# metacraft-labs/dvt-circuits

Measured on AMD Instinct MI355X. Metric: SP1 prover cycles/sec + proofs/hour, finalization_prove at 1/2/4/8 MI355X, higher is better.
Workload: dtype u32; 1 GPU; BASELINE configs[1] input: examples/finalization_test.json (tests/golden/finalization_example.json) through the reference's JSON -> CBOR -> SP1Stdin encoding, executed AND proven (the whole prove() call) by the finalization-shaped synthetic guest tests/guests.py:dkg_like(6180, 1545, 1): 32 shards of 2^21 RV32IM cycles; the reference's own guest ELF is prebuilt machine code and is not run (it would; stdin_bytes=2165, participants=3, curve_precompiles=False, fri_queries=100, pow_bits=16, log_blowup=1

## Files before the change

### dvt_circuits_amd/capi.py

```python
import ctypes as C
import json
import os
import subprocess

import numpy as np

HERE = os.path.dirname(os.path.abspath(__file__))
LIB_PATH = os.path.join(HERE, "libdvt_prover.so")
CSRC = os.path.join(HERE, "csrc")

DVT_OK, DVT_ERR_GUEST, DVT_ERR_INPUT, DVT_ERR_DEVICE, DVT_ERR_UNSUPPORTED, DVT_ERR_REJECTED = 0, 1, 2, 3, 4, 5
PATHS = {"default": 0, "rows": 1, "parts": 2}
SELECTORS = {"table": 0, "kernel": 1}
DVT_KEEP_NONE, DVT_KEEP_TREE, DVT_KEEP_FULL = 0, 1, 2
u32p = C.POINTER(C.c_uint32)
u8p = C.POINTER(C.c_uint8)


class DevMatrix(C.Structure):
    _fields_ = [("d_data", C.c_void_p), ("width", C.c_uint32), ("log_height", C.c_uint32)]


class HostTrace(C.Structure):
    _fields_ = [("chip_id", C.c_uint32), ("log_n", C.c_uint32), ("data", u32p)]
# ... 66 lines not shown
    lib.dvt_stage_bus_ledger_add.argtypes = [vp, vp, u32, vp, vp, u32, u32p, u32]
    lib.dvt_stage_bus_ledger_collect.argtypes = [vp, vp, u32, vp, vp, u32, u32p, u32]
    lib.dvt_stage_bus_ledger_add_tuple.argtypes = [vp, vp, u32, u32p, u32, C.c_int32, u32, u32]
    lib.dvt_stage_bus_ledger_close.argtypes = [vp, vp, u32p]
    lib.dvt_stage_bus_ledger_result.argtypes = [vp, vp, C.POINTER(BusTuple), sz, C.POINTER(sz), u32p]
    lib.dvt_stage_bus_ledger_free.argtypes = [vp, vp]
    lib.dvt_rv32_job_bus_tuples.argtypes = [vp, vp, vp, C.POINTER(BusTuple), sz, C.POINTER(sz), u32p]
    lib.dvt_debug_ledger_key.argtypes = [C.c_uint64, u32, u32, u32p]
    u64 = C.c_uint64
    lib.dvt_stage_hunt_cells.argtypes = [vp, C.c_char_p, u32, vp, vp, u32, u32p, u64, u32p, u32, u32, u32, u64, u32p, u8p]
    lib.dvt_stage_hunt_pairs.argtypes = [vp, C.c_char_p, u32, vp, vp, u32, u32p, u64, u32p, u32, u32p, u32, u32, u32, u32, u64,
                                         C.POINTER(Escape), sz, C.POINTER(u64), C.POINTER(u64)]
    lib.dvt_rv32_hunt_shard.argtypes = [vp, vp, vp, sz, u32, u64, u32p, u32, u32, u32p, u32, u32, u32, u32, u64, u32p, u8p,
                                        C.POINTER(Escape), sz, C.POINTER(u64), C.POINTER(u64)]
    lib.dvt_debug_ledger_key.restype = C.c_uint64
    lib.dvt_stage_hunt_join_new.argtypes = [vp, C.c_char_p, u64, u32p, u32, sz, sz, u32, C.POINTER(vp)]
    lib.dvt_stage_hunt_join_supply.argtypes = [vp, vp, u32, vp, vp, u32, u32p]
    lib.dvt_stage_hunt_join_add.argtypes = [vp, vp, u32, u32, vp, vp, u32, u32p, u32, u32, u32p, u32, u64]
    lib.dvt_stage_hunt_join_match.argtypes = [vp, vp, C.POINTER(JoinSummary)]
    lib.dvt_stage_hunt_join_result.argtypes = [vp, vp, C.POINTER(JoinCell), sz, C.POINTER(sz), C.POINTER(JoinCell), sz, C.POINTER(sz)]
    lib.dvt_stage_hunt_join_free.argtypes = [vp, vp]
    lib.dvt_rv32_hunt_join_job.argtypes = [vp, vp, vp, C.POINTER(JoinWindow), sz, u32p, u32, u64, u32p, u32, u32p, u32p, u64, sz, sz, u32,
                                           C.POINTER(JoinSummary), C.POINTER(JoinCell), sz, C.POINTER(sz), C.POINTER(JoinCell), sz, C.POINTER(sz)]
    lib.dvt_rv32_job_shard_chips.argtypes = [vp, sz]
    lib.dvt_rv32_job_shard_chips.restype = u32
    lib.dvt_rv32_job_shard_chip_shape.argtypes = [vp, sz, u32, u32p, u32p]
    lib.dvt_machine_setup.argtypes = [vp, C.c_char_p, C.POINTER(HostTrace), sz, C.POINTER(vp), C.POINTER(u8p), C.POINTER(sz)]
    lib.dvt_pk_free.argtypes = [vp, vp]
    lib.dvt_pk_free.restype = None
    lib.dvt_machine_prove.argtypes = [vp, vp, C.POINTER(HostTrace), sz, u32p, sz, C.POINTER(u8p), C.POINTER(sz)]
    lib.dvt_machine_verify.argtypes = [C.c_char_p, sz, C.c_char_p, sz, u32, u32, C.POINTER(C.c_char_p)]
    lib.dvt_prover_machine_verify.argtypes = [vp, C.c_char_p, sz, C.c_char_p, sz, u32, u32, C.POINTER(C.c_char_p)]
    lib.dvt_prover_verify.argtypes = [vp, C.c_char_p, sz, C.c_char_p, sz, u32, u32, C.POINTER(C.c_int32), C.POINTER(u8p), C.POINTER(sz), C.POINTER(C.c_char_p)]
    lib.dvt_prover_verify_times.argtypes = [vp, C.POINTER(C.c_double)]
    lib.dvt_stage_sponge_rows.argtypes = [vp, u32p, u32p, sz, u32p]
    lib.dvt_stage_verify_paths.argtypes = [vp, C.POINTER(PathChain), sz, u8p]
    lib.dvt_stage_multipath_nodes.argtypes = [u32, u32p, sz, u32p, sz, C.POINTER(sz)]
    lib.dvt_stage_verify_multipath.argtypes = [vp, u32, u32p, u32p, sz, u8p, u32p, u32p, sz, u32p, u8p]
    for fn in (lib.dvt_proof_compact, lib.dvt_proof_expand):
        fn.argtypes = [C.c_char_p, sz, C.c_char_p, sz, u32, u32, C.POINTER(u8p), C.POINTER(sz), C.POINTER(C.c_char_p)]
    lib.dvt_debug_compact_list_sweep.argtypes = [C.c_char_p, sz, C.c_char_p, sz, u32, u32, C.POINTER(u64), C.POINTER(u64), C.POINTER(C.c_char_p)]
    lib.dvt_last_stage_ms.argtypes = [vp, C.POINTER(C.c_float)]
    lib.dvt_setup.argtypes = [vp, C.c_char_p, sz, C.POINTER(vp), C.POINTER(u8p), C.POINTER(sz)]
    lib.dvt_execute.argtypes = [C.c_char_p, sz, C.POINTER(Buf), sz, C.c_uint64, C.POINTER(u8p), C.POINTER(sz), C.POINTER(Report), C.POINTER(C.c_char_p)]
    lib.dvt_execute_io.argtypes = [C.c_char_p, sz, C.POINTER(Buf), sz, C.c_uint64, C.POINTER(u8p), C.POINTER(sz), C.POINTER(u8p), C.POINTER(sz), C.POINTER(Report), C.POINTER(C.c_char_p)]
    lib.dvt_debug_exec_rate.argtypes = [C.c_char_p, sz, C.POINTER(Buf), sz, u32, C.c_int]
    lib.dvt_debug_exec_rate.restype = C.c_double
    lib.dvt_debug_p2_f64_selfcheck.argtypes = [u32, u32]
    lib.dvt_debug_p2_f64_selfcheck.restype = u64
    lib.dvt_debug_p2_f64_sbox_check.argtypes = [u32, u32, C.POINTER(C.c_double)]
    lib.dvt_debug_p2_f64_sbox_check.restype = u64
    lib.dvt_debug_ntt_group_check.argtypes = [u32, u32] + [C.POINTER(C.c_double)] * 3
    lib.dvt_debug_ntt_group_check.restype = u64
    lib.dvt_prove_core.argtypes = [vp, vp, C.POINTER(Buf), sz, C.POINTER(u8p), C.POINTER(sz), C.POINTER(Report)]
    lib.dvt_verify.argtypes = [C.c_char_p, sz, C.c_char_p, sz, u32, u32, C.POINTER(C.c_int32), C.POINTER(u8p), C.POINTER(sz), C.POINTER(C.c_char_p)]
    lib.dvt_rv32_prepare.argtypes = [vp, vp, C.POINTER(Buf), sz, C.POINTER(vp), C.POINTER(Report)]
    lib.dvt_rv32_prepare_part.argtypes = [vp, vp, C.POINTER(Buf), sz, sz, sz, C.POINTER(vp), C.POINTER(Report)]
    lib.dvt_rv32_header_words.restype = u32
    lib.dvt_rv32_job_exec_wait_seconds.argtypes = [vp]
    lib.dvt_rv32_job_exec_wait_seconds.restype = C.c_double
    lib.dvt_rv32_prove_job.argtypes = [vp, vp, vp, C.POINTER(u8p), C.POINTER(sz)]
    lib.dvt_job_free.argtypes = [vp, vp]
    lib.dvt_job_free.restype = None
    lib.dvt_rv32_debug_traces.argtypes = [C.c_char_p, sz, C.POINTER(Buf), sz, u32, u32, u32p, C.POINTER(u32p), C.POINTER(sz), C.POINTER(C.c_char_p)]
    lib.dvt_rv32_job_shards.argtypes = [vp]
    lib.dvt_rv32_job_shards.restype = sz
    lib.dvt_rv32_job_shard_member.argtypes = [vp, sz]
    lib.dvt_rv32_job_shard_member.restype = C.c_int
    lib.dvt_rv32_job_shard_device_rows.argtypes = [vp, sz]
    lib.dvt_rv32_job_shard_device_rows.restype = u32
    lib.dvt_rv32_job_shard_kept.argtypes = [vp, sz]
    lib.dvt_rv32_job_shard_kept.restype = C.c_int
    lib.dvt_rv32_job_shard_kept_bytes.argtypes = [vp, sz]
    lib.dvt_rv32_job_shard_kept_bytes.restype = C.c_uint64
    lib.dvt_debug_keep_plan.argtypes = [C.c_int, u64, u64, u64, u64, u64, u64, u64, C.c_int, C.c_int64, u64]
    lib.dvt_debug_keep_plan.restype = C.c_int
    lib.dvt_rv32_commit_shard.argtypes = [vp, vp, vp, sz, u32p]
    lib.dvt_rv32_challenges.argtypes = [C.c_char_p, sz, u32p, sz, u32p]
    lib.dvt_rv32_prove_shard.argtypes = [vp, vp, vp, sz, u32p, C.POINTER(u8p), C.POINTER(sz)]
    lib.dvt_rv32_assemble.argtypes = [vp, C.POINTER(C.c_char_p), C.POINTER(sz), sz, C.POINTER(u8p), C.POINTER(sz)]
    lib.dvt_rv32_debug_device_traces.argtypes = [vp, vp, vp, sz, C.POINTER(u32p), C.POINTER(sz)]
    lib.dvt_rv32_debug_poke_cell.argtypes = [vp, vp, sz, u32, u32, u32, u32]
    prof_out = [C.POINTER(u64), sz, C.POINTER(ProfileEdge), sz, C.POINTER(ProfileSyscall), sz, C.POINTER(ProfileOpcode), sz, C.POINTER(ProfileSummary)]
    lib.dvt_rv32_job_profile.argtypes = [vp, vp, vp, u32] + prof_out
    lib.dvt_execute_profile.argtypes = [C.c_char_p, sz, C.POINTER(Buf), sz, u64] + prof_out + [C.POINTER(Report), C.POINTER(C.c_char_p)]
    tree_out = [C.POINTER(CalltreeArc), sz, C.POINTER(CalltreeFunc), sz, C.POINTER(CalltreeSummary)]
    lib.dvt_rv32_job_calltree.argtypes = [vp, vp, vp, u32] + tree_out
    lib.dvt_rv32_job_calltree_times.argtypes = [vp, C.POINTER(C.c_double)]
    lib.dvt_execute_calltree.argtypes = [C.c_char_p, sz, C.POINTER(Buf), sz, u64] + tree_out + [C.POINTER(Report), C.POINTER(C.c_char_p)]
    mem_out = [C.POINTER(u64), sz, C.POINTER(MemoryPage), sz, C.POINTER(MemorySummary)]
    lib.dvt_rv32_job_memory.argtypes = [vp, vp, vp] + mem_out
    lib.dvt_execute_memory.argtypes = [C.c_char_p, sz, C.POINTER(Buf), sz, u64] + mem_out + [C.POINTER(Report), C.POINTER(C.c_char_p)]
    watch_io = [C.POINTER(WatchQuery), sz, sz, C.POINTER(WatchHit), C.POINTER(u64), C.POINTER(WatchSummary)]
    lib.dvt_rv32_job_watch.argtypes = [vp, vp, vp] + watch_io
    lib.dvt_rv32_job_watch_times.argtypes = [vp, C.POINTER(C.c_double)]
    lib.dvt_execute_watch.argtypes = [C.c_char_p, sz, C.POINTER(Buf), sz, u64, u32] + watch_io + [C.POINTER(Report), C.POINTER(C.c_char_p)]
    snap_io = [u32, u32, C.POINTER(SnapRange), sz, C.POINTER(SnapCell), C.POINTER(SnapCell), sz, C.POINTER(SnapFrame), sz, C.POINTER(SnapSummary)]
    lib.dvt_rv32_job_snapshot.argtypes = [vp, vp, vp] + snap_io
    lib.dvt_rv32_job_snapshot_times.argtypes = [vp, C.POINTER(C.c_double)]
    lib.dvt_execute_snapshot.argtypes = [C.c_char_p, sz, C.POINTER(Buf), sz, u64, u32] + snap_io + [C.POINTER(Report), C.POINTER(C.c_char_p)]
    origin_io = [u32, u32, u32, u32, u32, u32, C.POINTER(OriginNode), sz, C.POINTER(OriginEdge), sz, C.POINTER(OriginSummary)]
    lib.dvt_rv32_job_origin.argtypes = [vp, vp, vp] + origin_io
    lib.dvt_rv32_job_origin_times.argtypes = [vp, C.POINTER(C.c_double)]
    lib.dvt_execute_origin.argtypes = [C.c_char_p, sz, C.POINTER(Buf), sz, u64, u32] + origin_io + [C.POINTER(Report), C.POINTER(C.c_char_p)]
    diverge_io = [DivergePos, DivergePos, u64, u32, u32, sz, C.POINTER(DivergePair), C.POINTER(DivergePair), C.POINTER(DivergeReg), C.POINTER(DivergeSummary)]
    lib.dvt_rv32_job_diverge.argtypes = [vp, vp, vp, vp] + diverge_io
# ... 527 lines not shown
    first, last, regs, s = (DivergePair * max(keep, 1))(), (DivergePair * max(keep, 1))(), (DivergeReg * 32)(), DivergeSummary()
    rc = call(DivergePos(*start_a), DivergePos(*start_b), max_pairs, DVT_DIVERGE_REJOIN if rejoin else 0, window, keep, first, last, regs, C.byref(s))
    if rc != DVT_OK:
        return rc, None
    summary = {}
    for name, kind in DivergeSummary._fields_:
        if name in ("pad", "pad2"):
            continue
        v = getattr(s, name)
        if kind is DivergeRec:
            summary[name] = {k: int(getattr(v, k)) for k in _DIV_REC_KEYS if k != "valid"} if v.valid else None
        else:
            summary[name] = float(v) if name == "ms" else int(v)
    n = summary["n_kept"]
    return rc, dict(summary=summary, regs=[{k: int(getattr(regs[r], k)) for k in _DIV_REG_KEYS} for r in range(32)],
                    first=[{k: int(getattr(first[i], k)) for k in _DIV_PAIR_KEYS} for i in range(n)],
                    last=[{k: int(getattr(last[i], k)) for k in _DIV_PAIR_KEYS} for i in range(n)])


def execute_diverge(elf: bytes, stdin_a: bytes, stdin_b: bytes, start_a=DIVERGE_ENTRY, start_b=DIVERGE_ENTRY, max_pairs=0, rejoin=False, window=0, keep=16,
                    max_cycles=0, log_shard=21):
    lib = load()
    reps, err = (Report(), Report()), C.c_char_p()
    a, b = bytes(stdin_a), bytes(stdin_b)
    rc, got = _diverge(lambda *io: lib.dvt_execute_diverge(elf, len(elf), a, len(a), b, len(b), max_cycles, log_shard, *io, C.byref(reps[0]), C.byref(reps[1]),
                                                           C.byref(err)), start_a, start_b, max_pairs, rejoin, window, keep)
    return rc, tuple(dict(cycles=r.cycles, exit_code=r.exit_code, halted=bool(r.halted), unprovable=bool(r.unprovable)) for r in reps), got, _take_str(lib, err)


def exec_rate(elf: bytes, stdin=(), log_shard=21, trace=False) -> float:
    return float(load().dvt_debug_exec_rate(elf, len(elf), _bufs(stdin), len(stdin), log_shard, int(trace)))


def keep_plan(mode, free, total, reserve, full, tree, later, remaining=0, count_known=True, full_cap=-1, full_kept=0) -> int:
    return int(load().dvt_debug_keep_plan(mode, free, total, reserve, full, tree, later, remaining, int(bool(count_known)), full_cap, full_kept))


def p2_f64_selfcheck(n: int, seed: int) -> int:
    return int(load().dvt_debug_p2_f64_selfcheck(n, seed))


def p2_f64_sbox_check(n: int, seed: int):
    mx = (C.c_double * 4)()
    bad = load().dvt_debug_p2_f64_sbox_check(n, seed, mx)
    return int(bad), [float(v) for v in mx]


def ntt_group_check(n: int, seed: int):
    mx = [(C.c_double * 8)() for _ in range(3)]
    bad = load().dvt_debug_ntt_group_check(n, seed, *mx)
    return int(bad), {k: [float(v) for v in m] for k, m in zip(("dif", "dif_unit", "dit"), mx)}


def execute_io(elf: bytes, stdin=(), max_cycles=0):
    lib = load()
    pv, n, so, m, rep, err = u8p(), C.c_size_t(), u8p(), C.c_size_t(), Report(), C.c_char_p()
    rc = lib.dvt_execute_io(elf, len(elf), _bufs(stdin), len(stdin), max_cycles, C.byref(pv), C.byref(n), C.byref(so), C.byref(m), C.byref(rep), C.byref(err))
    out = C.string_at(pv, n.value) if pv else b""
    sout = C.string_at(so, m.value) if so else b""
    for ptr in (pv, so):
        if ptr:
            lib.dvt_free(C.cast(ptr, C.c_void_p))
    return rc, dict(cycles=rep.cycles, exit_code=rep.exit_code, halted=bool(rep.halted), unprovable=bool(rep.unprovable)), out, sout, _take_str(lib, err)


def stdin_from_json(circuit_type: str, json_bytes: bytes, auth_commitment=False) -> bytes:
    lib = load()
    out, n, err = u8p(), C.c_size_t(), C.c_char_p()
    rc = lib.dvt_stdin_from_json(circuit_type.encode(), json_bytes, len(json_bytes), int(bool(auth_commitment)), C.byref(out), C.byref(n), C.byref(err))
    if rc:
        raise DvtError(rc, _take_str(lib, err))
    b = C.string_at(out, n.value)
    lib.dvt_free(C.cast(out, C.c_void_p))
    return b


def verify(vk: bytes, proof: bytes, fri_queries=100, pow_bits=16):
    lib = load()
    ec, pv, n, why = C.c_int32(), u8p(), C.c_size_t(), C.c_char_p()
    rc = lib.dvt_verify(vk, len(vk), proof, len(proof), fri_queries, pow_bits, C.byref(ec), C.byref(pv), C.byref(n), C.byref(why))
    out = C.string_at(pv, n.value) if pv else b""
    if pv:
        lib.dvt_free(C.cast(pv, C.c_void_p))
    return rc == DVT_OK, ec.value, out, _take_str(lib, why)


def _transcode(fn, vk, proof, fri_queries, pow_bits):
    lib = load()
    out, n, why = u8p(), C.c_size_t(), C.c_char_p()
    rc = fn(vk, len(vk), proof, len(proof), fri_queries, pow_bits, C.byref(out), C.byref(n), C.byref(why))
    reason = _take_str(lib, why)
    if rc:
        raise DvtError(rc, reason)
    b = C.string_at(out, n.value)
    lib.dvt_free(C.cast(out, C.c_void_p))
    return b


def proof_compact(vk: bytes, proof: bytes, fri_queries=100, pow_bits=16) -> bytes:
    return _transcode(load().dvt_proof_compact, vk, proof, fri_queries, pow_bits)


def proof_expand(vk: bytes, proof: bytes, fri_queries=100, pow_bits=16) -> bytes:
    return _transcode(load().dvt_proof_expand, vk, proof, fri_queries, pow_bits)


# ... 627 lines not shown
```

### dvt_circuits_amd/csrc/capi_rv32.hip

```cpp
#include <algorithm>
#include <atomic>
#include <cstdio>
#include <deque>
#include <map>

#include "capi_job.h"
#include "ntt_group.cuh"
#include "poseidon2_f64.cuh"
#include "sha256.h"

using namespace dvt;
static_assert(DVT_KEEP_NONE == KEEP_NONE && DVT_KEEP_TREE == KEEP_TREE && DVT_KEEP_FULL == KEEP_FULL, "the tiers of include/dvt_prover.h");

namespace {
std::vector<std::vector<uint8_t>> collect_stdin(const dvt_buf *bufs, size_t n) {
    std::vector<std::vector<uint8_t>> v(n);
    for (size_t i = 0; i < n; i++)
        if (bufs[i].len) v[i].assign(bufs[i].data, bufs[i].data + bufs[i].len);
    return v;
}
uint8_t *dup_bytes(const std::vector<uint8_t> &v, size_t *len) {
    uint8_t *b = (uint8_t *)malloc(v.size() + 1);
    if (b && !v.empty()) memcpy(b, v.data(), v.size());
    if (len) *len = v.size();
    return b;
}
PermChallenges global_challenges(const VerifyingKey &vk, const uint32_t *headers, size_t n) {
    Challenger g;
    g.observe(vk.prep_root);
    g.observe_u32((uint32_t)n);
    for (size_t i = 0; i < n; i++) {
        const uint32_t *h = headers + i * HEADER_WORDS;
        for (uint32_t k = 0; k < 8; k++) g.observe(Fp::from_canonical(h[k]));
        g.observe_u32(N_PUB);
        for (uint32_t k = 0; k < N_PUB; k++) g.observe(Fp::from_canonical(h[8 + k] % P));
    }
    PermChallenges c;
    c.alpha = g.sample_ext();
    c.beta = g.sample_ext();
    return c;
}
void pv_digest_words(const std::vector<uint8_t> &pv, uint32_t out[8]) {
    uint8_t dg[32];
    sha256(pv.data(), pv.size(), dg);
    for (int k = 0; k < 8; k++) out[k] = dg[4 * k] | (dg[4 * k + 1] << 8) | (dg[4 * k + 2] << 16) | ((uint32_t)dg[4 * k + 3] << 24);
}
}

int dvt::same_members(dvt_prover *p, const dvt_pk *pk, const dvt_job *j) {
    const size_t G = n_members(p);
    if ((pk && pk->dev.size() != G) || (j && j->parts.size() != G)) return fail(p, DVT_ERR_INPUT, "proving key or job of a handle with other devices");
    return DVT_OK;
}

static void job_release(dvt_prover *p, dvt_job *j) {
    if (!j) return;
    for (size_t m = std::min(j->parts.size(), n_members(p)); m-- > 0;) {
        (void)turn_to(p, m);
        Member &mem = member(p, m);
// ... 1486 lines not shown
            if (kind == 2) {
                const int64_t a = ref[j], b = ref[j + dist] * wj % (int64_t)P;
                ref[j] = (a + b) % (int64_t)P; ref[j + dist] = ntg_mod(a - b);
            } else {
                const int64_t a = ref[j], b = ref[j + dist];
                ref[j] = (a + b) % (int64_t)P; ref[j + dist] = ntg_mod(a - b) * wj % (int64_t)P;
            }
        }
    }
    uint64_t bad = 0;
    for (int j = 0; j < 8; j++)
        for (int c = 0; c < 2; c++) {
            const double x = v[j][c];
            const bool sane = fabs(x) < 9e15 && x == floor(x);
            bad += !sane || ntg_mod((int64_t)x) != (c ? ntg_mod(-ref[j]) : ref[j]);
        }
    return bad;
}
}

uint64_t dvt_debug_ntt_group_check(uint32_t n, uint32_t seed, double *max_dif, double *max_dif_unit, double *max_dit) {
    uint64_t bad = 0, s = 0x9e3779b97f4a7c15ull ^ seed;
    double mx[3][8] = {};
    const int64_t lim[3] = {(int64_t)ntg::DIF_IN, (int64_t)ntg::DIF_IN, (int64_t)ntg::DIT_IN}, half = ((int64_t)P - 1) / 2;
    auto next = [&]() { s ^= s << 13; s ^= s >> 7; s ^= s << 17; return s; };
    auto uniform = [&](int64_t m) { return (int64_t)(next() % (2 * (uint64_t)m + 1)) - m; };
    int64_t in[8], tw[7];
    for (uint32_t g = 0; g < n; g++)
        for (int kind = 0; kind < 3; kind++) {
            for (int j = 0; j < 8; j++) in[j] = uniform(lim[kind]);
            for (int k = 0; k < 7; k++) tw[k] = uniform(half);
            bad += ntg_check_one(kind, in, tw, mx[kind]);
        }
    const int64_t mags[5] = {0, 1, half, (int64_t)P - 1, (int64_t)(0.52 * p2f::PD)};
    const int64_t tws[4] = {1, -1, half, -half};
    for (int kind = 0; kind < 3; kind++)
        for (int m = 0; m < 5; m++)
            for (int signs = 0; signs < 256; signs++) {
                if (m == 0 && signs) break;
                const int64_t mag = mags[m] > lim[kind] ? lim[kind] : mags[m];
                for (int j = 0; j < 8; j++) in[j] = (signs >> j) & 1 ? -mag : mag;
                for (int c = 0; c < 64 + 8; c++) {
                    for (int k = 0; k < 7; k++) {
                        const int stage = kind == 2 ? (k < 1 ? 0 : k < 3 ? 1 : 2) : (k < 4 ? 0 : k < 6 ? 1 : 2);
                        tw[k] = c < 64 ? tws[(c >> (2 * stage)) & 3] : uniform(half);
                    }
                    bad += ntg_check_one(kind, in, tw, mx[kind]);
                }
            }
    for (int k = 0; k < 8; k++) { max_dif[k] = mx[0][k]; max_dif_unit[k] = mx[1][k]; max_dit[k] = mx[2][k]; }
    return bad;
}

}
```

### dvt_circuits_amd/csrc/f64dot.cuh

```cuda
#pragma once
#include "poseidon2_f64.cuh"

namespace dvt {

struct DotAcc {
    double lo, hi;
    DVT_HD void add(double w, double vlo, double vhi) { lo = fma(w, vlo, lo); hi = fma(w, vhi, hi); }
    DVT_HD void reduce() { lo = p2f::red(lo); hi = p2f::red(hi); }
    DVT_HD Fp value() const { return Fp::raw(p2f::fix(p2f::red(fma(p2f::red(hi), 65536.0, lo)))); }
};
struct DotAcc4 {
    DotAcc c[4];
    DVT_HD DotAcc4() { for (int k = 0; k < 4; k++) c[k] = DotAcc{0.0, 0.0}; }
    DVT_HD void add(const double *w4, Fp v) {
        const double vlo = (double)(v.v & 0xffffu), vhi = (double)(v.v >> 16);
#pragma unroll
        for (int k = 0; k < 4; k++) c[k].add(w4[k], vlo, vhi);
    }
    DVT_HD void reduce() {
#pragma unroll
        for (int k = 0; k < 4; k++) c[k].reduce();
    }
    DVT_HD Fp4 value() const {
        Fp4 r;
#pragma unroll
        for (int k = 0; k < 4; k++) r.c[k] = c[k].value();
        return r;
    }
    DVT_HD void value_canonical(double out[4]) const {
#pragma unroll
        for (int k = 0; k < 4; k++) out[k] = p2f::mm(p2f::red(fma(p2f::red(c[k].hi), 65536.0, c[k].lo)), p2f::MONT_RINV);
    }
};
struct Fd4 {
    double c[4];
};
DVT_HD Fd4 operator*(const Fd4 &a, const Fd4 &b) {
    const double q0 = b.c[0] * p2f::PINV, q1 = b.c[1] * p2f::PINV, q2 = b.c[2] * p2f::PINV, q3 = b.c[3] * p2f::PINV;
    auto m = [&](int i, int j, double qj) { return p2f::mm_pre(a.c[i], b.c[j], qj); };
    Fd4 r;
    r.c[0] = fma(11.0, m(1, 3, q3) + m(2, 2, q2) + m(3, 1, q1), m(0, 0, q0));
    r.c[1] = fma(11.0, m(2, 3, q3) + m(3, 2, q2), m(0, 1, q1) + m(1, 0, q0));
    r.c[2] = fma(11.0, m(3, 3, q3), m(0, 2, q2) + m(1, 1, q1) + m(2, 0, q0));
    r.c[3] = (m(0, 3, q3) + m(1, 2, q2)) + (m(2, 1, q1) + m(3, 0, q0));
    return r;
}
DVT_HD Fd4 operator*(const Fd4 &a, double b) {
    const double bq = b * p2f::PINV;
    Fd4 r;
    for (int k = 0; k < 4; k++) r.c[k] = p2f::mm_pre(a.c[k], b, bq);
    return r;
}
DVT_HD Fd4 operator+(const Fd4 &a, const Fd4 &b) { Fd4 r; for (int k = 0; k < 4; k++) r.c[k] = a.c[k] + b.c[k]; return r; }
DVT_HD Fd4 operator-(const Fd4 &a, const Fd4 &b) { Fd4 r; for (int k = 0; k < 4; k++) r.c[k] = a.c[k] - b.c[k]; return r; }

DVT_HD double centred_from_mont(uint32_t m) { return p2f::from_mont(m); }

}
```

### dvt_circuits_amd/csrc/machine.h

```cpp
#pragma once
#include "check.cuh"
#include "stark.cuh"

namespace dvt {

struct VerifierAccess {
    const Fp4 *main_l, *main_n, *prep_l, *prep_n, *perm_l, *perm_n;
    const Fp *pubv;
    Fp4 main(int c, int r) const { return r ? main_n[c] : main_l[c]; }
    Fp4 prep(int c, int r) const { return r ? prep_n[c] : prep_l[c]; }
    Fp4 pub(int k) const { return Fp4::from_base(pubv[k]); }
    Fp4 perm(int e, int r) const {
        const Fp4 *p = (r ? perm_n : perm_l) + 4 * e;
        Fp4 acc = p[0];
        for (int k = 1; k < 4; k++) {
            Fp4 basis = Fp4::zero();
            basis.c[k] = Fp::one();
            acc += basis * p[k];
        }
        return acc;
    }
};

struct VerifierPoint {
    const Fp4 *alpha_pows, *beta_pows;
    Fp4 perm_alpha, cum_over_n, sel_first, sel_last, sel_trans;
};

struct LedgerArgs;
struct HuntArgs;
struct JoinArgs;

struct ChipDesc {
    const char *name;
    int main_w, prep_w, n_pub, n_constraints, n_interactions, max_arity;
    int perm_ext_w;
    int n_folded;
    bool perm_parts, quot_parts;
    hipError_t (*launch_perm)(hipStream_t, const PermArgs &);
    hipError_t (*launch_quotient)(hipStream_t, const QuotientArgs &);
    Fp4 (*verify_eval)(const VerifierAccess &, const VerifierPoint &);
    hipError_t (*launch_check)(hipStream_t, const CheckArgs &) = nullptr;
    hipError_t (*launch_bus)(hipStream_t, const BusArgs &) = nullptr;
    hipError_t (*launch_ledger)(hipStream_t, const LedgerArgs &) = nullptr;
    hipError_t (*launch_hunt)(hipStream_t, const HuntArgs &, unsigned row_blocks, unsigned n_candidates) = nullptr;
    hipError_t (*launch_join)(hipStream_t, const JoinArgs &, unsigned row_blocks, unsigned n_candidates) = nullptr;
    hipError_t (*launch_supply)(hipStream_t, const JoinArgs &) = nullptr;
};

struct MachineDesc {
    const char *name;
    int n_chips;
    const ChipDesc *chips;
};

constexpr int RV32_FIRST_WIDE_CHIP = 9;
const MachineDesc *machine_toy();
const MachineDesc *machine_rv32();
const MachineDesc *machine_by_name(const char *name);

#if defined(__HIPCC__)
template <class Air>
constexpr bool perm_parts_parallel() { return Air::N_INTERACTIONS > 0 && Air::N_LPARTS > 1 && Air::N_LPARTS <= PARTS_MAX; }
template <class Air>
constexpr bool quot_parts_parallel() {
    constexpr int NP = Air::N_PARTS + (Air::N_INTERACTIONS > 0 ? Air::N_LPARTS : 0);
    return NP > 2 && NP <= PARTS_MAX && Air::MAIN_W >= 128;
}
template <class Air>
hipError_t launch_perm_t(hipStream_t st, const PermArgs &a) {
    if (Air::N_INTERACTIONS == 0) return hipSuccess;
    size_t n = (size_t)1 << a.log_n;
    if constexpr (perm_parts_parallel<Air>()) {
        if (a.partial) {
            perm_rows_parts_kernel<Air><<<dim3((unsigned)((n + 255) / 256), Air::N_LPARTS), 256, 0, st>>>(a);
            sum_parts_kernel<0><<<(unsigned)((4 * n + 255) / 256), 256, 0, st>>>(a.partial, Air::N_LPARTS, 4 * n, a.totals);
            return hipGetLastError();
        }
    }
    perm_rows_kernel<Air><<<(unsigned)((n + 255) / 256), 256, 0, st>>>(a);
    return hipGetLastError();
}
template <class Air, int PART>
void launch_quotient_parts(hipStream_t st, const QuotientArgs &a, unsigned blocks) {
    constexpr int LAST = Air::N_PARTS + (Air::N_INTERACTIONS > 0 ? Air::N_LPARTS : 0) - 1;
    quotient_kernel<Air, PART><<<blocks, 256, 0, st>>>(a);
    if constexpr (PART < LAST) launch_quotient_parts<Air, PART + 1>(st, a, blocks);
}
template <class Air>
hipError_t launch_quotient_t(hipStream_t st, const QuotientArgs &a) {
    size_t m = (size_t)2 << a.log_n;
    constexpr int NP = Air::N_PARTS + (Air::N_INTERACTIONS > 0 ? Air::N_LPARTS : 0);
    if constexpr (quot_parts_parallel<Air>()) {
        if (a.partial) {
            quotient_parts_kernel<Air><<<dim3((unsigned)((m + 255) / 256), NP), 256, 0, st>>>(a);
            sum_parts_kernel<0><<<(unsigned)((4 * m + 255) / 256), 256, 0, st>>>(a.partial, NP, 4 * m, a.out);
            return hipGetLastError();
        }
    }
    launch_quotient_parts<Air, 0>(st, a, (unsigned)((m + 255) / 256));
    return hipGetLastError();
}
template <class Air>
Fp4 verify_eval_t(const VerifierAccess &ax, const VerifierPoint &pt) {
    ConstraintFolder<Air, Fp4, VerifierAccess> f(ax);
    f.alpha_pows = pt.alpha_pows;
    f.beta_pows = pt.beta_pows;
    f.perm_alpha = pt.perm_alpha;
    f.cum_over_n = pt.cum_over_n;
    f.sel_first = pt.sel_first;
    f.sel_last = pt.sel_last;
    f.sel_trans = pt.sel_trans;
    return f.run();
}
template <class Air>
constexpr ChipDesc make_chip_desc() {
    return ChipDesc{Air::NAME, Air::MAIN_W, Air::PREP_W, Air::N_PUB, Air::N_CONSTRAINTS, Air::N_INTERACTIONS,
                    Air::MAX_ARITY, PermShape<Air>::EXT_W, PermShape<Air>::N_FOLDED,
                    perm_parts_parallel<Air>(), quot_parts_parallel<Air>(), &launch_perm_t<Air>, &launch_quotient_t<Air>, &verify_eval_t<Air>};
}
template <class Air>
ChipDesc with_check_fns(ChipDesc d) {
    d.launch_check = &launch_check_t<Air>;
    d.launch_bus = &launch_bus_t<Air>;
    return d;
}
#endif

}
```

### dvt_circuits_amd/csrc/machine_rv32_wide.hip

```cpp
#include "machine.h"
#if !defined(__HIP_DEVICE_COMPILE__)
#pragma clang optimize off
#endif
#include "gen/air_rv32.inc"
#if !defined(__HIP_DEVICE_COMPILE__)
#pragma clang optimize on
#endif

#include "gen/rv32_cols.h"
static_assert(dvt::RV32_FIRST_WIDE_CHIP == RV32_CHIP_FP_OP, "machine.h RV32_FIRST_WIDE_CHIP must be the fp_op chip");

namespace dvt {
namespace {
template <int I, class A>
bool pick(int chip, ChipDesc *out) {
    if constexpr (I >= RV32_FIRST_WIDE_CHIP) {
        if (chip == I) { *out = make_chip_desc<A>(); return true; }
    }
    return false;
}
}
ChipDesc rv32_wide_chip_desc(int chip) {
    ChipDesc d{};
#define DVT_X(i, A) if (pick<i, A>(chip, &d)) return d;
    DVT_AIR_RV32_CHIPS(DVT_X)
#undef DVT_X
    return d;
}
}
```

### dvt_circuits_amd/csrc/stark.cuh

```cuda
#pragma once
#include "bb.cuh"
#include "f64dot.cuh"
#include "kernels.h"

namespace dvt {

constexpr int WHEN_ALL = 0, WHEN_FIRST = 1, WHEN_LAST = 2, WHEN_TRANS = 3;

DVT_HD Fp4 to_ext(Fp a) { return Fp4::from_base(a); }
DVT_HD Fp4 to_ext(const Fp4 &a) { return a; }

template <class Air>
struct PermShape {
    static constexpr int NB = (Air::N_INTERACTIONS + 1) / 2;
    static constexpr int EXT_W = Air::N_INTERACTIONS ? NB : 0;
    static constexpr int PHI = NB - 1;
    static constexpr int BASE_W = 4 * EXT_W;
    static constexpr int N_FOLDED = Air::N_CONSTRAINTS + (Air::N_INTERACTIONS ? NB : 0);
};

template <class Air, class TT, class Access>
struct ConstraintFolder {
    using T = TT;
    using Shape = PermShape<Air>;
// ... 126 lines not shown
        if ((j & 1) == 0) {
            pend_m = m;
            pend_d = d;
            if (j == Air::N_INTERACTIONS - 1) {
                Fp4 p = batch_value(j >> 1);
                fold(Air::N_CONSTRAINTS + (j >> 1), p * d - to_ext(m));
            }
        } else {
            Fp4 p = batch_value(j >> 1);
            Fp4 lhs = p * pend_d * d;
            Fp4 rhs = d * pend_m + pend_d * m;
            fold(Air::N_CONSTRAINTS + (j >> 1), lhs - rhs);
        }
    }

    template <int PART = -1>
    DVT_HD Fp4 run() {
        if constexpr (BASE)
            for (int k = 0; k < 4; k++) perm_alpha_c.c[k] = centred_from_mont(perm_alpha.c[k].v);
        if constexpr (PART < 0) {
            Air::constraints(*this);
            Air::interactions(*this);
        } else if constexpr (PART < Air::N_PARTS) {
            Air::template constraints_part<PART>(*this);
        } else {
            Air::template interactions_part<PART - Air::N_PARTS>(*this);
        }
        if constexpr (BASE) {
            acc += acc_d.value();
            Fp4 lc;
            for (int k = 0; k < 4; k++) lc.c[k] = Fp::raw(p2f::to_mont(acc_c.c[k]));
            acc += lc;
        }
        return acc;
    }
};

#if defined(__HIPCC__)
struct PermArgs {
    const uint32_t *main;
    const uint32_t *prep;
    const uint32_t *pub;
    uint32_t *perm;
    uint32_t *totals;
    const Fp4 *beta_pows;
    const double *beta_d;
    Fp4 perm_alpha;
    uint32_t log_n;
    uint32_t *partial = nullptr;
};
constexpr int PARTS_MAX = 32;
constexpr uint32_t PARTS_PARALLEL_LOG = 15;

template <class Air>
struct PermRowCtx {
    using T = Fp;
    const PermArgs &a;
    size_t n, row;
    Fp4 batch, total;
    __device__ PermRowCtx(const PermArgs &args, size_t r) : a(args), n((size_t)1 << args.log_n), row(r), batch(Fp4::zero()), total(Fp4::zero()) {}
    __device__ static T K(uint32_t m) { return Fp::raw(m); }
    __device__ static T KI(uint32_t canonical) { return Fp::from_canonical(canonical); }
    __device__ T main(int c, int r) const { return Fp::raw(a.main[(size_t)c * n + ((row + r) & (n - 1))]); }
    __device__ T prep(int c, int r) const { return Fp::raw(a.prep[(size_t)c * n + ((row + r) & (n - 1))]); }
    __device__ T pub(int k) const { return Fp::raw(a.pub[k]); }
    __device__ void store_ext(int extcol, const Fp4 &v) {
#pragma unroll
        for (int k = 0; k < 4; k++) a.perm[((size_t)(4 * extcol + k)) * n + row] = v.c[k].v;
    }
    __device__ void interaction(int j, int bus, int sign, int , const T &mult, const T *vals, int nv) {
        Fp4 term = Fp4::zero();
        if (!mult.is_zero()) {
            DotAcc4 s;
            for (int k = 0; k < nv; k++) {
                s.add(a.beta_d + 4 * k, vals[k]);
                if ((k & 31) == 31) s.reduce();
            }
            Fp4 d = a.perm_alpha + Fp::from_canonical((uint32_t)bus) + s.value();
            term = inv(d) * (sign > 0 ? mult : -mult);
        }
        if ((j & 1) == 0) batch = term; else batch += term;
        if ((j & 1) || j == Air::N_INTERACTIONS - 1) {
            if ((j >> 1) < PermShape<Air>::PHI) store_ext(j >> 1, batch);
            total += batch;
        }
    }
};

template <class Air>
__global__ void __launch_bounds__(256) perm_rows_kernel(PermArgs a) {
    size_t row = (size_t)blockIdx.x * blockDim.x + threadIdx.x;
    if (row >= ((size_t)1 << a.log_n)) return;
    PermRowCtx<Air> ctx(a, row);
    Air::interactions(ctx);
#pragma unroll
    for (int k = 0; k < 4; k++) a.totals[(size_t)k * ctx.n + row] = ctx.total.c[k].v;
}

template <class Air, int LP, class Ctx>
__device__ __forceinline__ void interactions_of_part(Ctx &ctx, int part) {
    if (part == LP) Air::template interactions_part<LP>(ctx);
    else if constexpr (LP + 1 < Air::N_LPARTS) interactions_of_part<Air, LP + 1>(ctx, part);
}
template <class Air>
__global__ void __launch_bounds__(256) perm_rows_parts_kernel(PermArgs a) {
    size_t row = (size_t)blockIdx.x * blockDim.x + threadIdx.x;
    if (row >= ((size_t)1 << a.log_n)) return;
    PermRowCtx<Air> ctx(a, row);
    interactions_of_part<Air, 0>(ctx, (int)blockIdx.y);
#pragma unroll
    for (int k = 0; k < 4; k++) a.partial[((size_t)blockIdx.y * 4 + k) * ctx.n + row] = ctx.total.c[k].v;
}
template <int UNUSED>
__global__ void __launch_bounds__(256) sum_parts_kernel(const uint32_t *partial, uint32_t nparts, size_t words, uint32_t *out) {
    size_t w = (size_t)blockIdx.x * blockDim.x + threadIdx.x;
    if (w >= words) return;
    Fp acc = Fp::raw(partial[w]);
    for (uint32_t p = 1; p < nparts; p++) acc = acc + Fp::raw(partial[(size_t)p * words + w]);
    out[w] = acc.v;
}

struct QuotientArgs {
    const uint32_t *main_lde;
    const uint32_t *prep_lde;
    const uint32_t *perm_lde;
    const uint32_t *pub;
    uint32_t *out;
    const Fp4 *alpha_pows;
    const Fp4 *beta_pows;
    const double *alpha_d, *beta_d;
    Fp4 perm_alpha, cum_over_n;
    Fp zinv_even, zinv_odd;
    Fp z_even, z_odd;
    Fp w_inv;
    uint32_t log_n;
    NttTables tabs;
    const uint32_t *sel = nullptr;
    uint32_t *partial = nullptr;
};

__device__ __forceinline__ void selectors_of_row(const QuotientArgs &a, size_t i, Fp *sel_first, Fp *sel_last, Fp *sel_trans) {
    const uint32_t log_m = a.log_n + 1;
    Fp x = Fp::raw(a.tabs.sh_lo[1]) * (Fp::raw(a.tabs.tw_hi[((uint32_t)i << (24 - log_m)) >> 12]) *
                                        Fp::raw(a.tabs.tw_lo[((uint32_t)i << (24 - log_m)) & 4095]));
    const Fp zh = (i & 1) ? a.z_odd : a.z_even;
    Fp d1 = x - Fp::one(), d2 = x - a.w_inv;
    Fp pinv = inv(d1 * d2);
    *sel_first = zh * (pinv * d2);
    *sel_last = zh * (pinv * d1);
    *sel_trans = d2;
}
template <int UNUSED>
__global__ void __launch_bounds__(256) selector_table_kernel(QuotientArgs a, uint32_t *out) {
    const size_t m = (size_t)2 << a.log_n;
    size_t i = (size_t)blockIdx.x * blockDim.x + threadIdx.x;
    if (i >= m) return;
    Fp f, l, t;
    selectors_of_row(a, i, &f, &l, &t);
    out[i] = f.v; out[m + i] = l.v; out[2 * m + i] = t.v;
}

// ... 81 lines not shown
```

### include/dvt_prover.h

```cpp
#ifndef DVT_PROVER_H
#define DVT_PROVER_H
#include <stddef.h>
#include <stdint.h>
#ifdef __cplusplus
extern "C" {
#endif

#define DVT_OK 0
#define DVT_ERR_GUEST 1
#define DVT_ERR_INPUT 2
#define DVT_ERR_DEVICE 3
#define DVT_ERR_UNSUPPORTED 4
#define DVT_ERR_REJECTED 5

typedef struct dvt_prover dvt_prover;
typedef struct dvt_pk dvt_pk;

int dvt_prover_create(const char *cfg_json, dvt_prover **out);
uint32_t dvt_prover_device_count(const dvt_prover *p);
int dvt_prover_device(const dvt_prover *p, uint32_t member);
void dvt_prover_destroy(dvt_prover *p);
const char *dvt_last_error(const dvt_prover *p);
void dvt_free(void *ptr);
uint32_t dvt_abi_version(void);
// ... 352 lines not shown
enum { DVT_DIV_RD = 1, DVT_DIV_RS1 = 2, DVT_DIV_RS2 = 4, DVT_DIV_MEM = 8 };
enum { DVT_DIVERGE_REJOIN = 1 };
enum { DVT_DIV_SPLIT = 1, DVT_DIV_BAD = 2, DVT_DIV_END_BOTH = 3, DVT_DIV_END_A = 4, DVT_DIV_END_B = 5, DVT_DIV_LIMIT = 6 };
typedef struct { uint32_t shard, row; } dvt_diverge_pos;
typedef struct { uint32_t valid, pc, idx, a, b, c, m_prev, pad; } dvt_diverge_rec;
typedef struct {
    uint64_t k;
    uint32_t shard_a, row_a, shard_b, row_b, idx, pc, mask, dir;
    uint32_t a_a, b_a, c_a, m_a, a_b, b_b, c_b, m_b;
    uint32_t addr_a, before_a, after_a, addr_b, before_b, after_b;
} dvt_diverge_pair;
typedef struct { uint64_t n_diff, first_diff, last_diff, last_write; uint32_t live, pad; } dvt_diverge_reg;
typedef struct {
    uint64_t n_pairs, n_data, first_data, last_data, n_load_diffs, n_store_diffs, launched_pairs, cycles_a, cycles_b;
    uint32_t reason, mask, stop_shard_a, stop_row_a, stop_shard_b, stop_row_b;
    uint32_t rejoin_shard_a, rejoin_row_a, rejoin_shard_b, rejoin_row_b, rejoin_skip_a, rejoin_skip_b;
    uint32_t n_kept, span, window, batch_pairs;
    dvt_diverge_rec stop_a, stop_b, prev_a, prev_b;
    float ms;
    uint32_t pad2;
} dvt_diverge_summary;
int dvt_rv32_job_diverge(dvt_prover *p, const dvt_pk *pk, dvt_job *job_a, dvt_job *job_b, dvt_diverge_pos start_a, dvt_diverge_pos start_b,
                         uint64_t max_pairs, uint32_t flags, uint32_t window, size_t cap_each, dvt_diverge_pair *first, dvt_diverge_pair *last,
                         dvt_diverge_reg regs[32], dvt_diverge_summary *summary);
int dvt_rv32_job_diverge_times(dvt_prover *p, double out[4]);
int dvt_execute_diverge(const uint8_t *elf, size_t elf_len, const uint8_t *stdin_a, size_t n_a, const uint8_t *stdin_b, size_t n_b, uint64_t max_cycles,
                        uint32_t log_shard_size, dvt_diverge_pos start_a, dvt_diverge_pos start_b, uint64_t max_pairs, uint32_t flags, uint32_t window,
                        size_t cap_each, dvt_diverge_pair *first, dvt_diverge_pair *last, dvt_diverge_reg regs[32], dvt_diverge_summary *summary,
                        dvt_report *report_a, dvt_report *report_b, char **err_text);
int dvt_rv32_debug_device_traces(dvt_prover *p, const dvt_pk *pk, dvt_job *job, size_t shard, uint32_t **blob,
                                 size_t *blob_words);
int dvt_rv32_debug_poke_cell(dvt_prover *p, dvt_job *job, size_t shard, uint32_t chip, uint32_t col, uint32_t row,
                             uint32_t add);
int dvt_verify(const uint8_t *vk, size_t vk_len, const uint8_t *proof, size_t proof_len, uint32_t fri_queries,
               uint32_t pow_bits, int32_t *exit_code, uint8_t **public_values, size_t *pv_len, char **reason);
int dvt_prover_verify(dvt_prover *p, const uint8_t *vk, size_t vk_len, const uint8_t *proof, size_t proof_len,
                      uint32_t fri_queries, uint32_t pow_bits, int32_t *exit_code, uint8_t **public_values,
                      size_t *pv_len, char **reason);
int dvt_proof_compact(const uint8_t *vk, size_t vk_len, const uint8_t *proof, size_t proof_len, uint32_t fri_queries,
                      uint32_t pow_bits, uint8_t **out, size_t *out_len, char **reason);
int dvt_proof_expand(const uint8_t *vk, size_t vk_len, const uint8_t *proof, size_t proof_len, uint32_t fri_queries,
                     uint32_t pow_bits, uint8_t **out, size_t *out_len, char **reason);
int dvt_debug_compact_list_sweep(const uint8_t *vk, size_t vk_len, const uint8_t *proof, size_t proof_len, uint32_t fri_queries,
                                 uint32_t pow_bits, uint64_t *n_words, uint64_t *n_accepted, char **reason);
int dvt_prover_verify_times(dvt_prover *p, double out[9]);
int dvt_debug_keep_plan(int mode, uint64_t free_bytes, uint64_t total_bytes, uint64_t reserve_bytes, uint64_t full_bytes,
                        uint64_t tree_bytes, uint64_t later_bytes, uint64_t remaining, int count_known, int64_t full_cap,
                        uint64_t full_kept);
double dvt_debug_exec_rate(const uint8_t *elf, size_t elf_len, const dvt_buf *stdin_bufs, size_t nbuf, uint32_t log_shard,
                           int trace);
uint64_t dvt_debug_p2_f64_selfcheck(uint32_t n, uint32_t seed);
uint64_t dvt_debug_p2_f64_sbox_check(uint32_t n, uint32_t seed, double *max_abs);
uint64_t dvt_debug_ntt_group_check(uint32_t n, uint32_t seed, double *max_dif, double *max_dif_unit, double *max_dit);
uint64_t dvt_debug_ledger_key(uint64_t seed, uint32_t bus, uint32_t arity, const uint32_t *values);

int dvt_stdin_from_json(const char *type, const char *json, size_t json_len, int auth_commitment, uint8_t **out,
                        size_t *out_len, char **err_text);
int dvt_json_schema_validate(const char *schema, size_t schema_len, const char *json, size_t json_len, char **err_text);

int dvt_rv32_debug_traces(const uint8_t *elf, size_t elf_len, const dvt_buf *stdin_bufs, size_t nbuf, uint32_t log_shard,
                          uint32_t shard, uint32_t *n_shards, uint32_t **blob, size_t *blob_words, char **err_text);

#ifdef __cplusplus
}
#endif
#endif
```

Measured before the change: 80.78 million guest cycles/s.

## Compute permutation interactions in f64 with paired-fraction batching for narrow chips

Adds an f64 path for the permutation (logup) row kernel on non-wide chips. Quartic-extension products and inverses are done in double-precision Montgomery arithmetic, and interactions are paired so that one extension inverse serves two fractions (d1*m2 + d2*m1)/(d1*d2). The aim is to cut the cost of per-interaction Fp4 inversions and integer Montgomery multiplies on the GPU. Wide chips keep the old integer path. It adds numerical-range risk in f64 and ships a host self-check for that.

```diff
diff --git a/dvt_circuits_amd/capi.py b/dvt_circuits_amd/capi.py
--- a/dvt_circuits_amd/capi.py
+++ b/dvt_circuits_amd/capi.py
@@ -142,6 +142,8 @@
     lib.dvt_debug_p2_f64_sbox_check.restype = u64
     lib.dvt_debug_ntt_group_check.argtypes = [u32, u32] + [C.POINTER(C.c_double)] * 3
     lib.dvt_debug_ntt_group_check.restype = u64
+    lib.dvt_debug_k45_f64_check.argtypes = [u32, u32, C.POINTER(C.c_double)]
+    lib.dvt_debug_k45_f64_check.restype = u64
     lib.dvt_prove_core.argtypes = [vp, vp, C.POINTER(Buf), sz, C.POINTER(u8p), C.POINTER(sz), C.POINTER(Report)]
     lib.dvt_verify.argtypes = [C.c_char_p, sz, C.c_char_p, sz, u32, u32, C.POINTER(C.c_int32), C.POINTER(u8p), C.POINTER(sz), C.POINTER(C.c_char_p)]
     lib.dvt_rv32_prepare.argtypes = [vp, vp, C.POINTER(Buf), sz, C.POINTER(vp), C.POINTER(Report)]
@@ -775,6 +777,12 @@
     return int(bad), {k: [float(v) for v in m] for k, m in zip(("dif", "dif_unit", "dit"), mx)}
 
 
+def k45_f64_check(n: int, seed: int):
+    mx = (C.c_double * 3)()
+    bad = load().dvt_debug_k45_f64_check(n, seed, mx)
+    return int(bad), [float(v) for v in mx]
+
+
 def execute_io(elf: bytes, stdin=(), max_cycles=0):
     lib = load()
     pv, n, so, m, rep, err = u8p(), C.c_size_t(), u8p(), C.c_size_t(), Report(), C.c_char_p()
diff --git a/dvt_circuits_amd/csrc/capi_rv32.hip b/dvt_circuits_amd/csrc/capi_rv32.hip
--- a/dvt_circuits_amd/csrc/capi_rv32.hip
+++ b/dvt_circuits_amd/csrc/capi_rv32.hip
@@ -5,6 +5,7 @@
 #include <map>
 
 #include "capi_job.h"
+#include "f64dot.cuh"
 #include "ntt_group.cuh"
 #include "poseidon2_f64.cuh"
 #include "sha256.h"
@@ -1597,4 +1598,70 @@
     return bad;
 }
 
-}
+uint64_t dvt_debug_k45_f64_check(uint32_t n, uint32_t seed, double *max_abs) {
+    uint64_t bad = 0, s = 0x9e3779b97f4a7c15ull ^ seed;
+    double mx[3] = {0, 0, 0};
+    const int64_t half = ((int64_t)P - 1) / 2;
+    auto next = [&]() { s ^= s << 13; s ^= s >> 7; s ^= s << 17; return s; };
+    auto uniform = [&](int64_t m) { return (int64_t)(next() % (2 * (uint64_t)m + 1)) - m; };
+    auto ref_of = [&](const Fd4 &a) {
+        Fp4 r;
+        for (int k = 0; k < 4; k++) r.c[k] = Fp::from_canonical((uint32_t)ntg_mod((int64_t)a.c[k]));
+        return r;
+    };
+    auto differs = [&](const Fd4 &got, const Fp4 &want, int slot) {
+        uint64_t d = 0;
+        for (int k = 0; k < 4; k++) {
+            const double x = got.c[k];
+            const bool sane = fabs(x) < 9e15 && x == floor(x);
+            d += !sane || (uint32_t)ntg_mod((int64_t)x) != want.c[k].canonical() || (fabs(x) < 1.4e14 && p2f::to_mont(x) != want.c[k].v);
+            if (sane) mx[slot] = fmax(mx[slot], fabs(x));
+        }
+        return d;
+    };
+    auto check_prod = [&](const Fd4 &a, const Fd4 &b) {
+        double am = 0, bm = 0;
+        for (int k = 0; k < 4; k++) { am = fmax(am, fabs(a.c[k])); bm = fmax(bm, fabs(b.c[k])); }
+        if (am * bm > FD4_PROD_IN) return;
+        mx[0] = fmax(mx[0], am * bm);
+        bad += differs(a * b, ref_of(a) * ref_of(b), 1);
+    };
+    auto check_inv = [&](const Fd4 &a) { bad += differs(inv(a), inv(ref_of(a)), 2); };
+    const int64_t wide = (int64_t)(6.12 * p2f::PD), mid = (int64_t)(1.02 * p2f::PD);
+    for (uint32_t t = 0; t < n; t++) {
+        Fd4 a, b;
+        for (int k = 0; k < 4; k++) { a.c[k] = (double)uniform(wide); b.c[k] = (double)uniform(mid); }
+        check_prod(a, b);
+        check_prod(b, a);
+        check_inv(b);
+        check_inv(a * b);
+        Fd4 c = b;
+        for (int k = 0; k < 4; k++) c.c[k] += (double)(uniform(16) * (int64_t)P);
+        check_inv(c);
+        check_inv(Fd4{{b.c[0], 0.0, 0.0, 0.0}});
+    }
+    const int64_t mags[7] = {0, 1, half, half + 1, (int64_t)P - 1, mid, wide};
+    for (int ma = 0; ma < 7; ma++)
+        for (int mb = 0; mb < 7; mb++)
+            for (int signs = 0; signs < 256; signs++) {
+                Fd4 a, b;
+                for (int k = 0; k < 4; k++) {
+                    a.c[k] = (double)((signs >> k) & 1 ? -mags[ma] : mags[ma]);
+                    b.c[k] = (double)((signs >> (4 + k)) & 1 ? -mags[mb] : mags[mb]);
+                }
+                check_prod(a, b);
+                if (mb == 0 && signs < 16) check_inv(a);
+            }
+    const int64_t singles[6] = {1, -1, half, -half, half + 1, -(half + 1)};
+    for (int k = 0; k < 4; k++)
+        for (int v = 0; v < 6; v++) {
+            Fd4 a = {{0.0, 0.0, 0.0, 0.0}};
+            a.c[k] = (double)singles[v];
+            check_inv(a);
+        }
+    for (int64_t z = -1; z <= 1; z++) check_inv(Fd4{{(double)(z * (int64_t)P), 0.0, (double)(-z * (int64_t)P), 0.0}});
+    for (int k = 0; k < 3; k++) max_abs[k] = mx[k];
+    return bad;
+}
+
+}
diff --git a/dvt_circuits_amd/csrc/f64dot.cuh b/dvt_circuits_amd/csrc/f64dot.cuh
--- a/dvt_circuits_amd/csrc/f64dot.cuh
+++ b/dvt_circuits_amd/csrc/f64dot.cuh
@@ -35,14 +35,16 @@
 struct Fd4 {
     double c[4];
 };
+constexpr int FD4_K = 12;
+constexpr double FD4_PROD_IN = 3.66e19;
 DVT_HD Fd4 operator*(const Fd4 &a, const Fd4 &b) {
     const double q0 = b.c[0] * p2f::PINV, q1 = b.c[1] * p2f::PINV, q2 = b.c[2] * p2f::PINV, q3 = b.c[3] * p2f::PINV;
-    auto m = [&](int i, int j, double qj) { return p2f::mm_pre(a.c[i], b.c[j], qj); };
+    auto m = [&](int i, int j, double qj) { return p2f::mm_c<FD4_K>(a.c[i], b.c[j], qj); };
     Fd4 r;
-    r.c[0] = fma(11.0, m(1, 3, q3) + m(2, 2, q2) + m(3, 1, q1), m(0, 0, q0));
-    r.c[1] = fma(11.0, m(2, 3, q3) + m(3, 2, q2), m(0, 1, q1) + m(1, 0, q0));
-    r.c[2] = fma(11.0, m(3, 3, q3), m(0, 2, q2) + m(1, 1, q1) + m(2, 0, q0));
-    r.c[3] = (m(0, 3, q3) + m(1, 2, q2)) + (m(2, 1, q1) + m(3, 0, q0));
+    r.c[0] = p2f::red(fma(11.0, m(1, 3, q3) + m(2, 2, q2) + m(3, 1, q1), m(0, 0, q0)));
+    r.c[1] = p2f::red(fma(11.0, m(2, 3, q3) + m(3, 2, q2), m(0, 1, q1) + m(1, 0, q0)));
+    r.c[2] = p2f::red(fma(11.0, m(3, 3, q3), m(0, 2, q2) + m(1, 1, q1) + m(2, 0, q0)));
+    r.c[3] = p2f::red((m(0, 3, q3) + m(1, 2, q2)) + (m(2, 1, q1) + m(3, 0, q0)));
     return r;
 }
 DVT_HD Fd4 operator*(const Fd4 &a, double b) {
@@ -54,6 +56,37 @@
 DVT_HD Fd4 operator+(const Fd4 &a, const Fd4 &b) { Fd4 r; for (int k = 0; k < 4; k++) r.c[k] = a.c[k] + b.c[k]; return r; }
 DVT_HD Fd4 operator-(const Fd4 &a, const Fd4 &b) { Fd4 r; for (int k = 0; k < 4; k++) r.c[k] = a.c[k] - b.c[k]; return r; }
 
+DVT_HD double inv_base(double a) {
+    const double ap = a * p2f::PINV;
+    const double a2 = p2f::mm_pre(a, a, ap), a3 = p2f::mm_pre(a2, a, ap);
+    const double a7 = p2f::mm_pre(p2f::mm(a3, a3), a, ap);
+    const double a7p = a7 * p2f::PINV;
+    double r = p2f::mm_pre(a7, a7, a7p);
+#pragma unroll
+    for (int i = 0; i < 9; i++) {
+        r = p2f::mm(r, r); r = p2f::mm(r, r); r = p2f::mm(r, r);
+        r = p2f::mm_pre(r, a7, a7p);
+    }
+    return r;
+}
+DVT_HD Fd4 inv(const Fd4 &a) {
+    using namespace p2f;
+    const double A0 = red(a.c[0]), B0 = red(a.c[1]), A1 = red(a.c[2]), B1 = red(a.c[3]);
+    const double A2_0 = fma(11.0, mm(A1, A1), mm(A0, A0)), A2_1 = 2.0 * mm(A0, A1);
+    const double B2_0 = fma(11.0, mm(B1, B1), mm(B0, B0)), B2_1 = 2.0 * mm(B0, B1);
+    const double D0 = fma(-11.0, B2_1, A2_0), D1 = A2_1 - B2_0;
+    const double ni = inv_base(fma(-11.0, mm(D1, D1), mm(D0, D0)));
+    const double nip = ni * PINV;
+    const double I0 = mm_pre(D0, ni, nip), I1 = -mm_pre(D1, ni, nip);
+    const double I0p = I0 * PINV, I1p = I1 * PINV;
+    Fd4 r;
+    r.c[0] = fma(11.0, mm_pre(A1, I1, I1p), mm_pre(A0, I0, I0p));
+    r.c[2] = mm_pre(A0, I1, I1p) + mm_pre(A1, I0, I0p);
+    r.c[1] = -fma(11.0, mm_pre(B1, I1, I1p), mm_pre(B0, I0, I0p));
+    r.c[3] = -(mm_pre(B0, I1, I1p) + mm_pre(B1, I0, I0p));
+    return r;
+}
+
 DVT_HD double centred_from_mont(uint32_t m) { return p2f::from_mont(m); }
 
 }
diff --git a/dvt_circuits_amd/csrc/machine.h b/dvt_circuits_amd/csrc/machine.h
--- a/dvt_circuits_amd/csrc/machine.h
+++ b/dvt_circuits_amd/csrc/machine.h
@@ -67,18 +67,21 @@
     constexpr int NP = Air::N_PARTS + (Air::N_INTERACTIONS > 0 ? Air::N_LPARTS : 0);
     return NP > 2 && NP <= PARTS_MAX && Air::MAIN_W >= 128;
 }
-template <class Air>
+struct ChipKind { static constexpr bool K4_F64 = true; };
+struct WideChipKind { static constexpr bool K4_F64 = false; };
+template <class Air, class Kind>
 hipError_t launch_perm_t(hipStream_t st, const PermArgs &a) {
+    constexpr bool F64 = Kind::K4_F64;
     if (Air::N_INTERACTIONS == 0) return hipSuccess;
     size_t n = (size_t)1 << a.log_n;
     if constexpr (perm_parts_parallel<Air>()) {
         if (a.partial) {
-            perm_rows_parts_kernel<Air><<<dim3((unsigned)((n + 255) / 256), Air::N_LPARTS), 256, 0, st>>>(a);
+            perm_rows_parts_kernel<Air, F64><<<dim3((unsigned)((n + 255) / 256), Air::N_LPARTS), 256, 0, st>>>(a);
             sum_parts_kernel<0><<<(unsigned)((4 * n + 255) / 256), 256, 0, st>>>(a.partial, Air::N_LPARTS, 4 * n, a.totals);
             return hipGetLastError();
         }
     }
-    perm_rows_kernel<Air><<<(unsigned)((n + 255) / 256), 256, 0, st>>>(a);
+    perm_rows_kernel<Air, F64><<<(unsigned)((n + 255) / 256), 256, 0, st>>>(a);
     return hipGetLastError();
 }
 template <class Air, int PART>
@@ -113,11 +116,11 @@
     f.sel_trans = pt.sel_trans;
     return f.run();
 }
-template <class Air>
+template <class Air, class Kind = ChipKind>
 constexpr ChipDesc make_chip_desc() {
     return ChipDesc{Air::NAME, Air::MAIN_W, Air::PREP_W, Air::N_PUB, Air::N_CONSTRAINTS, Air::N_INTERACTIONS,
                     Air::MAX_ARITY, PermShape<Air>::EXT_W, PermShape<Air>::N_FOLDED,
-                    perm_parts_parallel<Air>(), quot_parts_parallel<Air>(), &launch_perm_t<Air>, &launch_quotient_t<Air>, &verify_eval_t<Air>};
+                    perm_parts_parallel<Air>(), quot_parts_parallel<Air>(), &launch_perm_t<Air, Kind>, &launch_quotient_t<Air>, &verify_eval_t<Air>};
 }
 template <class Air>
 ChipDesc with_check_fns(ChipDesc d) {
diff --git a/dvt_circuits_amd/csrc/machine_rv32_wide.hip b/dvt_circuits_amd/csrc/machine_rv32_wide.hip
--- a/dvt_circuits_amd/csrc/machine_rv32_wide.hip
+++ b/dvt_circuits_amd/csrc/machine_rv32_wide.hip
@@ -15,7 +15,7 @@
 template <int I, class A>
 bool pick(int chip, ChipDesc *out) {
     if constexpr (I >= RV32_FIRST_WIDE_CHIP) {
-        if (chip == I) { *out = make_chip_desc<A>(); return true; }
+        if (chip == I) { *out = make_chip_desc<A, WideChipKind>(); return true; }
     }
     return false;
 }
diff --git a/dvt_circuits_amd/csrc/stark.cuh b/dvt_circuits_amd/csrc/stark.cuh
--- a/dvt_circuits_amd/csrc/stark.cuh
+++ b/dvt_circuits_amd/csrc/stark.cuh
@@ -202,13 +202,18 @@
 constexpr int PARTS_MAX = 32;
 constexpr uint32_t PARTS_PARALLEL_LOG = 15;
 
-template <class Air>
+template <class Air, bool F64 = true>
 struct PermRowCtx {
     using T = Fp;
     const PermArgs &a;
     size_t n, row;
     Fp4 batch, total;
-    __device__ PermRowCtx(const PermArgs &args, size_t r) : a(args), n((size_t)1 << args.log_n), row(r), batch(Fp4::zero()), total(Fp4::zero()) {}
+    Fd4 perm_alpha_c, pend_d;
+    double pend_m = 0.0;
+    __device__ PermRowCtx(const PermArgs &args, size_t r) : a(args), n((size_t)1 << args.log_n), row(r), batch(Fp4::zero()), total(Fp4::zero()) {
+        if constexpr (F64)
+            for (int k = 0; k < 4; k++) perm_alpha_c.c[k] = centred_from_mont(a.perm_alpha.c[k].v);
+    }
     __device__ static T K(uint32_t m) { return Fp::raw(m); }
     __device__ static T KI(uint32_t canonical) { return Fp::from_canonical(canonical); }
     __device__ T main(int c, int r) const { return Fp::raw(a.main[(size_t)c * n + ((row + r) & (n - 1))]); }
@@ -218,7 +223,56 @@
 #pragma unroll
         for (int k = 0; k < 4; k++) a.perm[((size_t)(4 * extcol + k)) * n + row] = v.c[k].v;
     }
+    __device__ static Fp4 to_mont4(const Fd4 &v) {
+        Fp4 r;
+#pragma unroll
+        for (int k = 0; k < 4; k++) r.c[k] = Fp::raw(p2f::to_mont(v.c[k]));
+        return r;
+    }
+    __device__ void interaction_f64(int j, int bus, int sign, const T &mult, const T *vals, int nv) {
+        double m = 0.0;
+        Fd4 d = {{1.0, 0.0, 0.0, 0.0}};
+        if (!mult.is_zero()) {
+            DotAcc4 s;
+            for (int k = 0; k < nv; k++) {
+                s.add(a.beta_d + 4 * k, vals[k]);
+                if ((k & 31) == 31) s.reduce();
+            }
+            Fd4 e;
+            s.value_canonical(e.c);
+            e.c[0] += (double)bus;
+            bool nz = false;
+#pragma unroll
+            for (int k = 0; k < 4; k++) {
+                e.c[k] = p2f::red(e.c[k] + perm_alpha_c.c[k]);
+                nz |= e.c[k] != 0.0;
+            }
+            if (nz) {
+                const double m0 = centred_from_mont(mult.v);
+                m = sign > 0 ? m0 : -m0;
+                d = e;
+            }
+        }
+        const bool tail = (j & 1) == 0 && j == Air::N_INTERACTIONS - 1;
+        if ((j & 1) == 0 && !tail) {
+            pend_m = m;
+            pend_d = d;
+            return;
+        }
+        batch = Fp4::zero();
+        if (tail) {
+            if (m != 0.0) batch = to_mont4(inv(d) * m);
+        } else if (m != 0.0 || pend_m != 0.0) {
+            batch = to_mont4((d * pend_m + pend_d * m) * inv(pend_d * d));
+        }
+        if ((j >> 1) < PermShape<Air>::PHI) store_ext(j >> 1, batch);
+        total += batch;
+    }
     __device__ void interaction(int j, int bus, int sign, int , const T &mult, const T *vals, int nv) {
+        if constexpr (F64) {
+            interaction_f64(j, bus, sign, mult, vals, nv);
+            return;
+        }
         Fp4 term = Fp4::zero();
         if (!mult.is_zero()) {
             DotAcc4 s;
@@ -237,11 +291,11 @@
     }
 };
 
-template <class Air>
+template <class Air, bool F64>
 __global__ void __launch_bounds__(256) perm_rows_kernel(PermArgs a) {
     size_t row = (size_t)blockIdx.x * blockDim.x + threadIdx.x;
     if (row >= ((size_t)1 << a.log_n)) return;
-    PermRowCtx<Air> ctx(a, row);
+    PermRowCtx<Air, F64> ctx(a, row);
     Air::interactions(ctx);
 #pragma unroll
     for (int k = 0; k < 4; k++) a.totals[(size_t)k * ctx.n + row] = ctx.total.c[k].v;
@@ -252,11 +306,11 @@
     if (part == LP) Air::template interactions_part<LP>(ctx);
     else if constexpr (LP + 1 < Air::N_LPARTS) interactions_of_part<Air, LP + 1>(ctx, part);
 }
-template <class Air>
+template <class Air, bool F64>
 __global__ void __launch_bounds__(256) perm_rows_parts_kernel(PermArgs a) {
     size_t row = (size_t)blockIdx.x * blockDim.x + threadIdx.x;
     if (row >= ((size_t)1 << a.log_n)) return;
-    PermRowCtx<Air> ctx(a, row);
+    PermRowCtx<Air, F64> ctx(a, row);
     interactions_of_part<Air, 0>(ctx, (int)blockIdx.y);
 #pragma unroll
     for (int k = 0; k < 4; k++) a.partial[((size_t)blockIdx.y * 4 + k) * ctx.n + row] = ctx.total.c[k].v;
diff --git a/include/dvt_prover.h b/include/dvt_prover.h
--- a/include/dvt_prover.h
+++ b/include/dvt_prover.h
@@ -428,6 +428,7 @@
 uint64_t dvt_debug_p2_f64_selfcheck(uint32_t n, uint32_t seed);
 uint64_t dvt_debug_p2_f64_sbox_check(uint32_t n, uint32_t seed, double *max_abs);
 uint64_t dvt_debug_ntt_group_check(uint32_t n, uint32_t seed, double *max_dif, double *max_dif_unit, double *max_dit);
+uint64_t dvt_debug_k45_f64_check(uint32_t n, uint32_t seed, double *max_abs);
 uint64_t dvt_debug_ledger_key(uint64_t seed, uint32_t bus, uint32_t arity, const uint32_t *values);
 
 int dvt_stdin_from_json(const char *type, const char *json, size_t json_len, int auth_commitment, uint8_t **out,
```

After: 80.85 million guest cycles/s, median of 2. No clear change (+0.1%).
